# ywrt/slam-robot

Hardware: AMD Instinct MI355X
Metric: local-BA iters/sec (50 KF, 20k pts) (higher is better)
Workload: dtype f64

## Files before the change

slam-robot_amd/csrc/ba_chol.hip:

```cpp
#include "ba_lm.h"
#include "ba_tile.h"

namespace sg {

constexpr int kPanelWaves = 3;

__device__ __forceinline__ double& Wn(double* win, int i, int j) {
  return win[(i & (kCholWS - 1)) * kCholLd + (j & (kCholWS - 1))];
}

__device__ __forceinline__ double readlane_d(double v, int l) {
  const int lo = __builtin_amdgcn_readlane(__double2loint(v), l);
  const int hi = __builtin_amdgcn_readlane(__double2hiint(v), l);
  return __hiloint2double(hi, lo);
}



__device__ __forceinline__ void chol_diag16(double (&col)[kCholNb], int w, int lane, bool& bad) {
#pragma unroll
  for (int j = 0; j < kCholNb; ++j) {
    if (j < w) {
      const double piv = readlane_d(col[j], j);
      if (!(piv > 0.0)) bad = true;
// ... 848 lines not shown

struct TileSrc {
  int rev;
  int np;
  int sep;
  int nb;
  int ld;
};

__device__ __forceinline__ f64x4 tile_load(const double* __restrict__ S, int I, int J, int li, int lk,
                                           const TileSrc& ts) {
  f64x4 t;
  const int n = ts.nb, ld = ts.ld;
  const int cz = ld * ld + ld;
  const bool zsep = I >= ts.sep && J >= ts.sep;
#pragma unroll
  for (int q = 0; q < 4; ++q) {
    const int gi = 16 * I + lk + 4 * q, gj = 16 * J + li;
    const int si = ts.rev ? ts.np - 1 - gj : gi, sj = ts.rev ? ts.np - 1 - gi : gj;
    const bool in = I >= 0 && si < n && sj < n && !zsep;
    t[q] = S[in ? si * ld + sj : cz + ((gi == gj && !zsep) ? 1 : 0)];
  }
  return t;
}


__device__ __forceinline__ bool tile_diag(const f64x4& D, double ypart, TileShared& sh, double* zp, int K,
                                          int lane, int li, int lk) {
#pragma unroll
  for (int q = 0; q < 4; ++q) sh.Dw[(lk + 4 * q) * kTLd + li] = (lk + 4 * q <= li) ? D[q] : 0.0;
  const double ys = sum_rows4(ypart);
  if (lk == 0) sh.Yw[li] = ys;
  double ca[kCholNb];
#ifdef SG_X_NOFACTOR
  const bool bad = false;
#pragma unroll
  for (int r = 0; r < kCholNb; ++r) ca[r] = sh.Dw[r * kTLd + (lane & 15)];
#else
  const bool bad = tile_factor(sh.Dw, sh.Yw, sh.Id, sh.prw, ca);
#endif
  double* Zs = sh.Zs[K & 3];
  double* zk = sh.zK[K & 3];
  if (lane >= 16 && lane < 32) {
#pragma unroll
    for (int r = 0; r < kCholNb; ++r) Zs[r * kTLd + (lane - 16)] = ca[r];
  }
  if (lane == 32) {
#pragma unroll
    for (int r = 0; r < kCholNb; ++r) zk[r] = ca[r];
  }
  return bad;
}

__device__ __forceinline__ void tile_zp(const TileShared& sh, double* zp, int K, int lane, double* zg = nullptr) {
  if (lane < 16) {
    const double* Zs = sh.Zs[K & 3];
    const double* zk = sh.zK[K & 3];
    double s = 0.0;
#pragma unroll
    for (int r = 0; r < kCholNb; ++r) s = fma(Zs[r * kTLd + lane], zk[r], s);
    zp[16 * K + lane] = s;
  }
  if (zg) {
    const double* Zs = sh.Zs[K & 3];
    double* dst = zg + (size_t)K * kTB * 256;
#pragma unroll
    for (int e = lane; e < 256; e += 64) dst[e] = Zs[(e >> 4) * kTLd + (e & 15)];
  }
}

#define SG_TSTAMP(slot)                                                                  \
  if (kStamp && lane == 0) {                                                             \
    const unsigned long long now_ = __builtin_amdgcn_s_memtime();                       \
    tacc[slot] += now_ - tlast;                                                          \
    tlast = now_;                                                                        \
  }
#ifdef SG_X_ARRIVE
#define SG_PTRACE(K, slot) {}
#undef SG_TSTAMP
#define SG_TSTAMP(slot) {}
#define SG_AST(slot)                                                             \
  if (kStamp && lane == 0) {                                                     \
    const unsigned long long now_ = __builtin_amdgcn_s_memtime();               \
    tacc[slot] += now_ - tlast;                                                  \
    tlast = now_;                                                                \
  }
#else
#define SG_AST(slot) {}
#define SG_PTRACE(K, slot)                                                                  \
  if (kStamp && lane == 0 && (K) < kTraceK)                                                \
    d.stamps[64 + ((size_t)blockIdx.x * kTraceK + (K)) * 16 + (slot)] = __builtin_amdgcn_s_memtime();
#endif

__device__ __forceinline__ f64x4 tile_w(const f64x4& U, const double* Zs, int li, int lk) {
  const f64x4 zero = {0.0, 0.0, 0.0, 0.0};
  double zt[4];
#pragma unroll
  for (int s = 0; s < 4; ++s) zt[s] = Zs[(4 * s + lk) * kTLd + li];
  return mfma_f64_k16(zt, U, zero);
}
__device__ __forceinline__ void tile_w_store(const f64x4& Wt, double* __restrict__ Wg, int K, int J, int lane) {
  double* wg = Wg + ((size_t)K * kTB + (J - K)) * 256 + lane;
#pragma unroll
  for (int q = 0; q < 4; ++q) wg[q * 64] = Wt[q];
}

__device__ __forceinline__ void tile_rotate(f64x4 (&acc)[kTB]) {
  const f64x4 t = acc[0];
#pragma unroll
  for (int u = 0; u < kTB - 1; ++u) acc[u] = acc[u + 1];
  acc[kTB - 1] = t;
}

__device__ __forceinline__ void tile_col_load(f64x4 (&acc)[kTB], double& ypart, const Dev& d, int J, int K,
                                              int li, int lk, const TileSrc& ts) {
#pragma unroll
  for (int u = 0; u < kTB; ++u) acc[u] = tile_load(d.S, J - ((J - (u + K - 1)) & 7), J, li, lk, ts);
  const int gj = 16 * J + li, ld = ts.ld;
  const int sj = ts.rev ? ts.np - 1 - gj : gj;
  ypart = d.S[(lk == 0 && sj < ts.nb && J < ts.sep) ? ld * ld + sj : ld * ld + ld];
}

constexpr int kLaSpinMax = 1 << 20;
__device__ __forceinline__ bool la_done(const int* tend, int Kp) {
  return Kp >= 0 && Kp + 2 < tend[Kp];
}

template <bool kStamp>
__device__ __forceinline__ void tile_phase(f64x4 (&acc)[kTB], double& ypart, int& J, bool& late, bool& bad,
                                           bool& tmo, TileShared& sh, const Dev& d,
                                           double* __restrict__ Wg, double* zp, const int* tend, int K, int NT,
                                           int lane, int li, int lk, const TileSrc& ts, double* zg,
                                           unsigned long long (&tacc)[16], unsigned long long& tlast) {
  if (late) {
#ifdef SG_X_NOLATE
    J += kTB;
    late = false;
    return;
#endif
    const bool hasw = J < tend[K - 1];
    f64x4 Wt = {0.0, 0.0, 0.0, 0.0};
    if (hasw) Wt = tile_w(acc[0], sh.Zs[(K - 1) & 3], li, lk);
    SG_AST(0)
    const int Jw = J;
    J += kTB;
#ifndef SG_X_NOLOAD
    tile_col_load(acc, ypart, d, J, K, li, lk, ts);
#endif
    SG_AST(1)
    if (hasw) tile_w_store(Wt, Wg, K - 1, Jw, lane);
    SG_AST(2)
    tile_zp(sh, zp, K, lane, zg);
    SG_AST(3)
    late = false;
    SG_TSTAMP(13)
    return;
  }
  if (J == K + 1) SG_PTRACE(K, 8)
#ifdef SG_X_PRIO
  if (J == K + 1) __builtin_amdgcn_s_setprio(3);
#endif
#ifdef SG_X_IDLE
  if (J != K + 1) return;
#endif
#ifdef SG_X_NOTRAIL
  if (K >= 1 && J < tend[K - 1] && J == K + 1) {
#else
  if (K >= 1 && J < tend[K - 1]) {
#endif
    const double* Ub = sh.Ur[(K - 1) & 1][0];
    const bool own_la = J == K + 1 && la_done(tend, K - 1);
#pragma unroll
    for (int dd = 1; dd < kTB; ++dd) {
      if (K - 1 + dd <= J && !(dd == 2 && J == K + 1) && !(dd == 1 && own_la)) {
        double a[4];
#pragma unroll
        for (int s = 0; s < 4; ++s) a[s] = -Ub[(dd - 1) * 256 + s * 64 + lane];
        acc[dd] = mfma_f64_k16(a, acc[0], acc[dd]);
      }
    }
  }
  SG_TSTAMP(8)
  if (J == K + 1) { SG_AST(5) } else { SG_AST(10) }
  if (J == K + 1) SG_PTRACE(K, 9)
  const int te = tend[K];
  const bool act = J < te;
  const double* Zs = sh.Zs[K & 3];
  if (act) {
    const f64x4 zero = {0.0, 0.0, 0.0, 0.0};
    double za[4];
#pragma unroll
    for (int s = 0; s < 4; ++s) za[s] = Zs[li * kTLd + 4 * s + lk];
    const f64x4 U = mfma_f64_k16(za, acc[1], zero);
    acc[1] = U;
    double* ur = sh.Ur[K & 1][J - K - 1];
#pragma unroll
    for (int q = 0; q < 4; ++q) ur[q * 64 + lane] = U[q];
    if (J == K + 1) {
      __builtin_amdgcn_fence(__ATOMIC_RELEASE, "workgroup");
      if (lane == 0) __hip_atomic_store(&sh.uflag, K, __ATOMIC_RELAXED, __HIP_MEMORY_SCOPE_WORKGROUP);
    }
    const double* zk = sh.zK[K & 3];
#pragma unroll
    for (int q = 0; q < 4; ++q) ypart = fma(-U[q], zk[lk + 4 * q], ypart);
    if (J == K + 2) {
      double a[4];
#pragma unroll
      for (int s = 0; s < 4; ++s) a[s] = -U[s];
      acc[3] = mfma_f64_k16(a, U, acc[3]);
      if (la_done(tend, K)) {
        int spin = 0;
        while (__hip_atomic_load(&sh.uflag, __ATOMIC_RELAXED, __HIP_MEMORY_SCOPE_WORKGROUP) < K &&
               ++spin < kLaSpinMax)
          __builtin_amdgcn_s_sleep(0);
        tmo |= spin >= kLaSpinMax;
        __builtin_amdgcn_fence(__ATOMIC_ACQUIRE, "workgroup");
        const double* U1 = sh.Ur[K & 1][0];
        double b1[4];
#pragma unroll
        for (int s = 0; s < 4; ++s) b1[s] = -U1[s * 64 + lane];
        acc[2] = mfma_f64_k16(b1, U, acc[2]);
      }
    }
  }
  SG_TSTAMP(9)
  if (J == K + 1) { SG_AST(6) } else { SG_AST(11) }
  if (J == K + 1) {
    SG_PTRACE(K, 10)
    if (act) {
      double a[4];
#pragma unroll
      for (int s = 0; s < 4; ++s) a[s] = -acc[1][s];
      acc[2] = mfma_f64_k16(a, acc[1], acc[2]);
    }
    SG_TSTAMP(10)
    SG_AST(7)
    SG_PTRACE(K, 11)
    if (K + 1 < NT) {
      bad |= tile_diag(acc[2], ypart, sh, zp, K + 1, lane, li, lk);
    }
    SG_AST(8)
#ifdef SG_X_PRIO
    __builtin_amdgcn_s_setprio(0);
#endif
    SG_PTRACE(K, 12)
    late = true;
    SG_TSTAMP(11)
  } else if (act) {
    tile_w_store(tile_w(acc[1], Zs, li, lk), Wg, K, J, lane);
    SG_AST(12)
    SG_TSTAMP(12)
  }
}

__device__ __forceinline__ void tile_final(f64x4 (&acc)[kTB], int J, bool& late, TileShared& sh,
                                           double* __restrict__ Wg, const int* tend, int K, int lane, int li,
                                           int lk) {
  if (late) {
    if (J < tend[K - 1]) tile_w_store(tile_w(acc[0], sh.Zs[(K - 1) & 3], li, lk), Wg, K - 1, J, lane);
    late = false;
    return;
  }
  if (J < tend[K - 1]) {
    const double* Ub = sh.Ur[(K - 1) & 1][0];
    const bool own_la = J == K + 1 && la_done(tend, K - 1);
#pragma unroll
    for (int dd = 1; dd < kTB; ++dd) {
      if (K - 1 + dd <= J && !(dd == 2 && J == K + 1) && !(dd == 1 && own_la)) {
        double a[4];
#pragma unroll
        for (int s = 0; s < 4; ++s) a[s] = -Ub[(dd - 1) * 256 + s * 64 + lane];
        acc[dd] = mfma_f64_k16(a, acc[0], acc[dd]);
      }
    }
  }
}

__device__ __forceinline__ void sep_write(const f64x4 (&acc)[kTB], double ypart, int J, int ND, int NT, int m,
                                          int ns, double* __restrict__ sepb, double* __restrict__ sepy, int li,
                                          int lk) {
  if (J < ND || J >= ND + ns) return;
  const double ys = sum_rows4(ypart);
  const int Io = NT - 1 - J;
#pragma unroll
  for (int u = 0; u < kTB; ++u) {
    const int I = J - ((J - (u + ND - 1)) & 7);
    if (I >= ND) {
      double* dst = sepb + ((Io - m) * 7 + (NT - 1 - I - m)) * 256;
      const int C0 = 15 - li;
#pragma unroll
      for (int q = 0; q < 4; ++q) {
        const int Rd = C0, Cd = 15 - (lk + 4 * q);
        dst[(Rd >> 2) * 64 + Cd + 16 * (Rd & 3)] = acc[u][q];
      }
    }
  }
  if (lk == 0) sepy[(Io - m) * 16 + 15 - li] = ys;
}

__device__ __forceinline__ void sep_merge(f64x4 (&acc)[kTB], double& ypart, int J, int m, int ns,
                                          const double* __restrict__ sepb, const double* __restrict__ sepy,
                                          int lane, int li, int lk) {
  if (J < m || J >= m + ns) return;
#pragma unroll
  for (int u0 = 0; u0 < kTB; u0 += 2) {
    f64x4 t[2];
    bool use[2];
#pragma unroll
    for (int h = 0; h < 2; ++h) {
      const int u = u0 + h;
      const int I = J - ((J - (u + m - 2)) & 7);
      use[h] = I >= m;
      const double* src = sepb + (use[h] ? ((I - m) * 7 + (J - m)) * 256 : 0) + lane;
#pragma unroll
      for (int q = 0; q < 4; ++q) t[h][q] = src[q * 64];
    }
#pragma unroll
    for (int h = 0; h < 2; ++h)
      if (use[h])
#pragma unroll
        for (int q = 0; q < 4; ++q) acc[u0 + h][q] += t[h][q];
  }
  if (lk == 0) ypart += sepy[(J - m) * 16 + li];
}

template <int kCtrl>
__device__ __forceinline__ double dpp_mv(double v) {
  const int lo = __builtin_amdgcn_mov_dpp(__double2loint(v), kCtrl, 0xF, 0xF, false);
  const int hi = __builtin_amdgcn_mov_dpp(__double2hiint(v), kCtrl, 0xF, 0xF, false);
  return __hiloint2double(hi, lo);
}
__device__ __forceinline__ double bs_rowsum(const double (&p)[4], bool b0, bool b1) {
  const double k0 = b0 ? p[2] : p[0], k1 = b0 ? p[3] : p[1];
  const double s0 = b0 ? p[0] : p[2], s1 = b0 ? p[1] : p[3];
  const double a0 = k0 + dpp_mv<0xB1>(s0), a1 = k1 + dpp_mv<0xB1>(s1);
  const double k = b1 ? a1 : a0, sd = b1 ? a0 : a1;
  double v = k + dpp_mv<0x4E>(sd);
  v += dpp_mv<0x124>(v);
  v += dpp_mv<0x128>(v);
  return v;
}
__device__ __forceinline__ int bs_src_lane(int li) {
  const int q = li >> 2;
  return (((q >> 1) & 1) | ((q & 1) << 1)) + 16 * (li & 3);
}

__device__ __forceinline__ void tile_diag_pre(const f64x4& Z, double ypart, TileShared& sh, int li, int lk) {
  double* Zs = sh.Zs[0];
#pragma unroll
  for (int q = 0; q < 4; ++q) Zs[(lk + 4 * q) * kTLd + li] = Z[q];
  const double y = sum_rows4(ypart);
  double p[4];
#pragma unroll
  for (int q = 0; q < 4; ++q) p[q] = Z[q] * y;
  int lb = li;
  asm volatile("" : "+v"(lb));
  const double tot = bs_rowsum(p, (lb & 1) != 0, (lb & 2) != 0);
  if (li < 4) sh.zK[0][lk + 4 * (2 * (li & 1) + ((li >> 1) & 1))] = tot;
}

#ifndef SG_BS_BUF
#define SG_BS_BUF 2
#endif
constexpr int kBsBuf = SG_BS_BUF;
template <bool kRev>
__device__ __forceinline__ void bs_chain(const double* __restrict__ Wb, const double* zsrc, double* xs, int Khi,
                                         int Klo, double (&xw)[kTB - 1], int NT, int lane, int li, int lk) {
  auto wload = [&](double (&w)[kTB - 1][4], int K) {
#ifdef SG_X_BSHOT
    const double* src = Wb + (size_t)0 * (K >= 0 ? K : 0) + lane;
#else
    const double* src = Wb + (size_t)(K >= 0 ? K : 0) * kTB * 256 + lane;
#endif
#pragma unroll
    for (int dd = 1; dd < kTB; ++dd)
#pragma unroll
// ... 86 lines not shown
#pragma unroll
      for (int q = 0; q < 4; ++q) p[q] = fma(w[dd - 1][q], xw[dd - 1], p[q]);
#pragma unroll
    for (int q = 0; q < 4; ++q) {
      double v = p[q];
      v += dpp_d<0xB1>(v);
      v += dpp_d<0x4E>(v);
      v += dpp_d<0x141>(v);
      v += dpp_d<0x140>(v);
      p[q] = zk[q] - v;
    }
    unsigned long long mb = 0ull;
#pragma unroll
    for (int q = 0; q < 4; ++q) {
      int msk;
      asm volatile("v_bfe_i32 %0, %1, %2, 1" : "=v"(msk) : "v"(qbits), "n"(q));
      mb |= (unsigned long long)__double_as_longlong(p[q]) & (unsigned long long)(long long)msk;
    }
    const double xk = __shfl(__longlong_as_double((long long)mb), srcl);
    xat(K) = xk;
    asm volatile("" ::: "memory");
    if (lane == 0) __hip_atomic_store(done + K, 1, __ATOMIC_RELAXED, __HIP_MEMORY_SCOPE_WORKGROUP);
    xown = xk;
    wload(w, K - 4);
  };
  const int K0 = Khi - par;
  if (K0 < Klo) return;
  double wA[kTB - 1][4], wB[kTB - 1][4], zA[4], zB[4];
  wload(wA, K0);
  wload(wB, K0 - 2);
#pragma unroll
  for (int q = 0; q < 4; ++q) zA[q] = zsrc[16 * K0 + lk + 4 * q];
  int K = K0;
  bool first = true;
  for (; K >= Klo + 2; K -= 4) {
#pragma unroll
    for (int q = 0; q < 4; ++q) zB[q] = zsrc[16 * (K - 2) + lk + 4 * q];
    bs_row(K, wA, zA, first);
    first = false;
#pragma unroll
    for (int q = 0; q < 4; ++q) zA[q] = zsrc[16 * (K >= 4 ? K - 4 : 0) + lk + 4 * q];
    bs_row(K - 2, wB, zB, false);
  }
  if (K >= Klo) bs_row(K, wA, zA, first);
}

constexpr int kSepSpinMax = 1 << 22;
template <bool kStamp>
__global__ __launch_bounds__(kTileThreads) void k_chol_tiles(Dev d, const int32_t* panel_jend,
                                                             double* __restrict__ Wg, int32_t* tflag, int nd,
                                                             int flags) {
  const LmState* st = d.st;
  unsigned long long tlast = kStamp ? __builtin_amdgcn_s_memtime() : 0ull, tacc[16] = {};
  __shared__ TileShared sh;
  extern __shared__ double tdyn[];
  const bool border = (flags & 8) != 0;
  const int n = border ? d.kc0 : d.n, tid = threadIdx.x, lane = tid & 63;
  const int wave = __builtin_amdgcn_readfirstlane(tid >> 6);
  const int li = lane & 15, lk = lane >> 4;
  const int NT = (n + 15) >> 4;
  const bool bottom = nd > 0 && blockIdx.x == 1;
  const int nsf = (flags >> 8) & 15;
  const int ns = nsf > 0 && nsf < kTB ? nsf : kTB - 1;
  const int m = nd > 0 ? NT - nd - ns : NT;
  const int NTf = nd > 0 ? (bottom ? nd : m + ns) : NT;
  double* Wb = bottom ? Wg + (size_t)NT * kTB * 256 : Wg;
  double* zpg = Wg + (size_t)2 * NT * kTB * 256;
  double* sepb = zpg + 16 * NT;
  double* sepy = sepb + 49 * 256;
  const TileSrc ts{bottom ? 1 : 0, 16 * NT, bottom ? nd : (1 << 28), n, d.n};
  double* zg = border ? Wb : nullptr;
  double* xs = tdyn;
  double* zp = tdyn + 16 * NT;
  int* tend = reinterpret_cast<int*>(tdyn + 32 * NT);
  int* rdone = tend + NT;
  int* rdone_b = rdone + NT;
  for (int k = tid; k < 2 * NT; k += kTileThreads) rdone[k] = 0;
  const bool cand_lds = (flags & 2) != 0;
  CandLds cl;
  cl.carve(tdyn + 32 * NT + (3 * NT + 1) / 2, d.F, d.D, n);
  const int epoch = (nd > 0 && !bottom) ? tflag[1] : 0;
  if (tid == 0) {
    sh.fail = 0;
    sh.tmo = 0;
    sh.uflag = -1;
  }
  bool bad = false, tmo = false;
  const int spin_max = (flags & 4) ? 256 : kSepSpinMax;
  if (bottom && (flags & 4))
    for (int i = 0; i < 640; ++i) __builtin_amdgcn_s_sleep(127);
  const bool zpre_in = (flags & 16) != 0 && !bottom;
  f64x4 D0;
  bool zbad = false;
  if (zpre_in) {
#pragma unroll
    for (int q = 0; q < 4; ++q) D0[q] = d.zpre[(lk + 4 * q) * 16 + li];
    zbad = d.zpre[256] != 0.0;
  } else {
    D0 = tile_load(d.S, 0, 0, li, lk, ts);
  }
  double y0;
  {
    const int sj0 = ts.rev ? ts.np - 1 - li : li, ld = ts.ld;
    y0 = d.S[(lk == 0 && sj0 < n && 0 < ts.sep) ? ld * ld + sj0 : ld * ld + ld];
  }
  const int done = st->done;
  if (lane == 0) sh.simd[wave] = __builtin_amdgcn_s_getreg((1 << 11) | (4 << 6) | 4);
  for (int i = tid; i < 16 * kTLd; i += kTileThreads) sh.Id[i] = (i / kTLd == i % kTLd) ? 1.0 : 0.0;
  lds_barrier();
  int col = wave;
  {
    const int my = sh.simd[wave];
    int cnt[4] = {0, 0, 0, 0}, rank = 0;
#pragma unroll
    for (int w = 0; w < kTB; ++w) {
      const int sw = sh.simd[w] & 3;
      cnt[sw] += 1;
      if (w < wave && sw == my) rank += 1;
    }
#ifdef SG_X_PAIR4
    if (cnt[0] == 2 && cnt[1] == 2 && cnt[2] == 2 && cnt[3] == 2) col = my + 4 * rank;
#else
    if (cnt[0] == 2 && cnt[1] == 2 && cnt[2] == 2 && cnt[3] == 2) col = 2 * my + rank;
#endif
  }
  {
    f64x4 acc[kTB];
    double ypart = 0.0;
    int J = col;
    bool late = false;
    if (J == 0) J = kTB;
    tile_col_load(acc, ypart, d, J, 0, li, lk, ts);
    for (int k = tid; k < NT; k += kTileThreads) {
      if (!bottom) {
        tend[k] = min((panel_jend[k] + 15) >> 4, NTf);
      } else {
        const int c = NT - 1 - k;
        int te[kTB];
#pragma unroll
        for (int h = 0; h < kTB; ++h) te[h] = panel_jend[max(0, c - kTB + h)];
        int lo = c;
#pragma unroll
        for (int h = kTB - 1; h >= 0; --h) {
          const int i = c - kTB + h;
          if (i >= 0 && ((te[h] + 15) >> 4) > c) lo = i;
        }
        tend[k] = min(NT - lo, nd + ns);
      }
    }
    if (done) return;
    if (col == 0) {
      if (zpre_in) {
        tile_diag_pre(D0, y0, sh, li, lk);
        bad |= zbad;
      } else {
        bad |= tile_diag(D0, y0, sh, zp, 0, lane, li, lk);
      }
      tile_zp(sh, zp, 0, lane, zg);
    }
    else if (cand_lds)
      cand_prefetch(d, cl, st->cur, (col - 1) * 64 + lane, kTileThreads - 64);
    SG_TSTAMP(0)
    __syncthreads();
    SG_TSTAMP(1)
#ifdef SG_X_ARRIVE
    unsigned long long ar_sum[8] = {}, ar_max[8] = {}, ar_cnt[8] = {};
    unsigned long long t_ph = __builtin_amdgcn_s_memtime();
#endif
#pragma nounroll
    for (int K = 0; K < NTf; ++K) {
#ifdef SG_X_ARRIVE
      const int d0 = min(max(J - K, 0), 7);
      const int role = late ? 0 : (J == K + 1 ? 1 : 2);
#endif
      if (nd > 0 && !bottom && K == m - 1) {
        int spin = 0;
        while (__hip_atomic_load(tflag, __ATOMIC_RELAXED, __HIP_MEMORY_SCOPE_AGENT) <= epoch &&
               ++spin < spin_max)
          __builtin_amdgcn_s_sleep(1);
        __builtin_amdgcn_fence(__ATOMIC_ACQUIRE, "agent");
        tmo |= spin >= spin_max;
        sep_merge(acc, ypart, J, m, ns, sepb, sepy, lane, li, lk);
      }
      tile_phase<kStamp>(acc, ypart, J, late, bad, tmo, sh, d, Wb, zp, tend, K, NTf, lane, li, lk, ts, zg,
                         tacc, tlast);
      SG_TSTAMP(2)
      if (!late) tile_rotate(acc);
      SG_PTRACE(K, wave)
#ifdef SG_X_ARRIVE
      if (role == 0) { SG_AST(4) } else if (role == 1) { SG_AST(9) } else { SG_AST(13) }
      if (kStamp) {
        const unsigned long long ta = __builtin_amdgcn_s_memtime() - t_ph;
#pragma unroll
        for (int q = 0; q < 8; ++q)
          if (q == d0) {
            ar_sum[q] += ta;
            ar_max[q] = ar_max[q] > ta ? ar_max[q] : ta;
            ar_cnt[q] += 1;
          }
      }
#endif
      lds_barrier();
      if (late) tile_rotate(acc);
#ifdef SG_X_ARRIVE
      t_ph = __builtin_amdgcn_s_memtime();
      tlast = t_ph;
#endif
      SG_TSTAMP(3)
    }
#ifdef SG_X_ARRIVE
    if (kStamp && lane == 0) {
      unsigned long long* o = reinterpret_cast<unsigned long long*>(d.stamps) + kSegStamp + blockIdx.x * 256 + wave * 24;
#pragma unroll
      for (int q = 0; q < 8; ++q) {
        o[q] += ar_sum[q];
        o[8 + q] = o[8 + q] > ar_max[q] ? o[8 + q] : ar_max[q];
        o[16 + q] += ar_cnt[q];
      }
      unsigned long long* o2 = reinterpret_cast<unsigned long long*>(d.stamps) + kSegStamp + 512 + blockIdx.x * 256 +
                               wave * 16;
#pragma unroll
      for (int q = 0; q < 16; ++q) o2[q] += tacc[q];
    }
#endif
    if (bottom) {
      tile_final(acc, J, late, sh, Wb, tend, nd, lane, li, lk);
      sep_write(acc, ypart, J, nd, NT, m, ns, sepb, sepy, li, lk);
    }
  }
  if (bottom) {
    if (bad && lane == 0) sh.fail = 1;
    __syncthreads();
    for (int i = tid; i < 16 * nd; i += kTileThreads) zpg[i] = zp[i];
    if (tid == 0) zpg[16 * nd] = sh.fail ? 1.0 : 0.0;
    __builtin_amdgcn_fence(__ATOMIC_RELEASE, "agent");
    __syncthreads();
    if (tid == 0) {
      const int c = tflag[0];
      __hip_atomic_store(tflag, c + 1, __ATOMIC_RELEASE, __HIP_MEMORY_SCOPE_AGENT);
    }
    return;
  }
  if (nd > 0 && zpg[16 * nd] != 0.0) bad = true;
  if (bad && lane == 0) sh.fail = 1;
  __syncthreads();
  SG_TSTAMP(4)
  const int cur = st->cur;
  {
    double xw[kTB - 1];
#pragma unroll
    for (int dd = 0; dd < kTB - 1; ++dd) xw[dd] = 0.0;
    constexpr int kBs2Rows = 12;
    if (nd == 0) {
      if (NT >= kBs2Rows) {
        if (wave < 2) bs_chain2<false>(Wg, zp, xs, rdone, NT - 1, 0, xw, NT, wave, lane, li, lk, tmo);
      } else if (wave == 0) {
        bs_chain<false>(Wg, zp, xs, NT - 1, 0, xw, NT, lane, li, lk);
      }
    } else {
      if (wave == 0) bs_chain<false>(Wg, zp, xs, m + ns - 1, m, xw, NT, lane, li, lk);
      __syncthreads();
      if (wave < 2) {
#pragma unroll
        for (int dd = 1; dd < kTB; ++dd) xw[dd - 1] = dd <= ns ? xs[16 * (m - 1 + dd) + li] : 0.0;
        if (m >= kBs2Rows)
          bs_chain2<false>(Wg, zp, xs, rdone, m - 1, 0, xw, NT, wave, lane, li, lk, tmo);
        else if (wave == 0)
          bs_chain<false>(Wg, zp, xs, m - 1, 0, xw, NT, lane, li, lk);
      } else if (wave < 4) {
#pragma unroll
        for (int dd = 1; dd < kTB; ++dd) xw[dd - 1] = dd <= ns ? xs[16 * (NT - nd - dd) + 15 - li] : 0.0;
        if (nd >= kBs2Rows)
          bs_chain2<true>(Wg + (size_t)NT * kTB * 256, zpg, xs, rdone_b, nd - 1, 0, xw, NT, wave - 2, lane, li,
                          lk, tmo);
        else if (wave == 2)
          bs_chain<true>(Wg + (size_t)NT * kTB * 256, zpg, xs, nd - 1, 0, xw, NT, lane, li, lk);
      }
    }
  }
  if (tid == 0 && nd > 0) tflag[1] = epoch + 1;
  if (bad && lane == 0) sh.fail = 1;
  if (tmo && lane == 0) sh.tmo = 1;
  SG_TSTAMP(5)
  __syncthreads();
  double* y = d.work;
  for (int i = tid; i < n; i += kTileThreads) {
    d.xc[i] = xs[i];
    y[i] = xs[i];
  }
  if (border) {
    if (tid == 0) {
      d.xchg_chol[kCFail] = sh.fail ? 1.0 : 0.0;
      d.xchg_chol[kCTimeout] = sh.tmo ? 1.0 : 0.0;
    }
    return;
  }
  if (!cand_lds) __syncthreads();
  if (cand_lds)
    chol_candidates_lds<kTileThreads>(d, xs, sh.fail, cl, cur, sh.tmo);
  else
    chol_candidates<kTileThreads>(d, xs, sh.fail, sh.tmo);
  SG_TSTAMP(6)
  if (kStamp && lane == 0 && wave < 2)
    for (int s_ = 0; s_ < 16; ++s_) d.stamps[16 * wave + s_] += tacc[s_];
}
#undef SG_TSTAMP

template <bool kQlds>
__global__ __launch_bounds__(kBordThreads) void k_chol_border(Dev d, double* __restrict__ Wg, int flags) {
  const LmState* st = d.st;
  if (st->done) return;
  extern __shared__ double bdyn[];
  const int n = d.n, nf = d.kc0, nk = n - nf, NT = (nf + 15) >> 4;
  const int tid = threadIdx.x, lane = tid & 63, wave = tid >> 6, li = lane & 15, lk = lane >> 4;
  const bool cand_lds = (flags & 2) != 0;
  double* xs = bdyn;
  double* zq = bdyn + 16 * NT;
  int* rdone = reinterpret_cast<int*>(bdyn + 32 * NT);
  size_t off = 32 * (size_t)NT + (NT + 1) / 2;
  constexpr bool qlds = kQlds;
  double* Ql = bdyn + off;
  double* Qg = Wg + (size_t)NT * kTB * 256;
  if (qlds) off += 256 * (size_t)NT;
  CandLds cl;
  cl.carve(bdyn + off, d.F, d.D, n);
  const double* S = d.S;
  const double* xc = d.xc;
  __shared__ double Cs[16][kTLd];
  __shared__ double rk[16], xk[16], rpart[kBordThreads / 64][16];
  __shared__ double Ids[16 * kTLd], prw[2 * kCholNb];
  for (int i = tid; i < 16 * kTLd; i += kBordThreads) Ids[i] = (i / kTLd == i % kTLd) ? 1.0 : 0.0;
  __shared__ int bad_sh;
  unsigned long long tst[10];
  auto now_t = []() {
    unsigned long long t;
    asm volatile("s_memtime %0\n\ts_waitcnt lgkmcnt(0)" : "=s"(t) : : "memory");
    return t;
  };
  tst[0] = now_t();
  auto bstamp = [&](int k) { tst[k + 1] = now_t(); };
  for (int k = 1; k < 10; ++k) tst[k] = tst[0];
  const int fail0 = d.xchg_chol[kCFail] != 0.0, tmo0 = d.xchg_chol[kCTimeout] != 0.0;
  for (int k = tid; k < NT; k += kBordThreads) rdone[k] = 0;
  if (tid == 0) bad_sh = fail0;
  __shared__ double vring[8][256], wring[4][256], fring[2][4][256];
  __shared__ int vpost, fpost[2], wdone;
  if (tid == 0) {
    vpost = -1;
    fpost[0] = fpost[1] = -1;
    wdone = -1;
  }
  __syncthreads();
  bool tmo_chain = false;
  auto wait_ge = [&](int* flag, int v) {
    int spin = 0;
    while (__hip_atomic_load(flag, __ATOMIC_RELAXED, __HIP_MEMORY_SCOPE_WORKGROUP) < v && ++spin < kLaSpinMax)
      __builtin_amdgcn_s_sleep(0);
// ... 298 lines not shown
```

slam-robot_amd/csrc/ba_plan.cpp:

```cpp
#include "ba_plan.h"

#include <algorithm>
#include <climits>
#include <utility>

#include "common.h"

namespace sg {


void PlanBlocks(const sg_problem& p, Order* o) {
  o->F = p.num_frames;
  o->P = p.num_points;
  o->M = p.num_obs;
  o->D = p.num_dist;
  o->frame_block.assign(o->F, -1);
  o->NB = 0;
  for (int f = 0; f < o->F; ++f)
    if (p.frame_rot_free[f] || p.frame_trans_free[f]) o->frame_block[f] = o->NB++;
  o->nk = p.cameras_free ? 7 * p.num_cameras : 0;
  o->n = 6 * o->NB + o->nk;
}

void PlanPointOrder(const sg_problem& p, Order* o) {
// ... 484 lines not shown
  std::vector<int32_t> panel_bend(std::max(npanel, 1), 0);
  for (int pk = 0; pk < npanel; ++pk) {
    const int row_hi = std::min(n, (pk + 1) * kCholNb) - 1;
    const int blk_hi = row_hi / 6;
    int jmax = (pk + 1) * kCholNb;
    for (int b = 0; b < NB; ++b)
      if (lo_blk[b] <= blk_hi) jmax = std::max(jmax, 6 * b + 6);
    jmax = std::min(jmax, n);
    panel_jmax[pk] = std::min(n, (jmax + kCholNb - 1) / kCholNb * kCholNb);
    if (nk) {
      panel_bend[pk] = std::min(jmax, 6 * NB);
      panel_jmax[pk] = n;
    }
  }
  if (nk) panel_jmax.insert(panel_jmax.end(), panel_bend.begin(), panel_bend.end());
  e.pack_off.assign(npanel + 1, 0);
  for (int pk = 0; pk < npanel; ++pk)
    e.pack_off[pk + 1] = e.pack_off[pk] + std::min(kCholNb, n - pk * kCholNb) * (panel_jmax[pk] - pk * kCholNb);
  e.npack = (size_t)e.pack_off[npanel] + n;
  e.band_tiles = 0;
  for (int pk = 0; pk < npanel; ++pk)
    e.band_tiles = std::max(e.band_tiles, (panel_jmax[pk] + kCholNb - 1) / kCholNb - pk);
  std::vector<int32_t>&stile = e.stile, &s_loff = e.s_loff, &s_lidx = e.s_lidx;
  const int nft = (6 * NB + kCholNb - 1) / kCholNb;
  std::vector<int32_t> row_off(nft + 1, 0), cend(nft, 0);
  for (int R = 0; R < nft; ++R) {
    cend[R] = std::min(nft, (panel_jmax[R] + kCholNb - 1) / kCholNb);
    row_off[R + 1] = row_off[R] + std::max(0, cend[R] - R);
    for (int C = R; C < cend[R]; ++C) stile.push_back((R << 16) | C);
  }
  std::vector<std::vector<int32_t>> tl(stile.size());
  for (int s = 0; s < nseg; ++s) {
    const SchurSeg& sg = segs[s];
    for (int u = 0; u < sg.ntw * (sg.ntw + 1) / 2; ++u) {
      const int R = sg.t0 + schur_tile_r(u), C = sg.t0 + schur_tile_c(u);
      if (R < nft && C < cend[R]) tl[row_off[R] + C - R].push_back(sg.s_off + 256 * u);
    }
  }
  size_t smax = 0;
  for (const auto& l : tl) smax = std::max(smax, l.size());
  e.s_lstride = (int)std::max<size_t>(256, (smax + 255) / 256 * 256);
  s_lidx.assign(std::max<size_t>(tl.size(), 1) * e.s_lstride, 0);
  for (size_t t = 0; t < tl.size(); ++t) {
    s_loff.push_back((int)tl[t].size());
    std::copy(tl[t].begin(), tl[t].end(), s_lidx.begin() + t * e.s_lstride);
  }
  e.nstile = (int)stile.size();
  if (stile.empty()) stile.push_back(0);
  if (s_loff.empty()) s_loff.push_back(0);
  return e;
}


CholPlan PlanChol(const Order& o, const Envelope& e, const CholGrants& g, const LoadKnobs& k) {
  const int F = o.F, D = o.D, n = o.n, NB = o.NB, nk = o.nk, npanel = e.npanel;
  const std::vector<int32_t>& panel_jmax = e.panel_jmax;
  CholPlan c;
  c.gstage = (size_t)std::max(n, 1) * 8 * (1 + kCholNb) <= g.global && k.chol_gstage;
  c.window = npanel <= kJendSh;
  for (int pk = 0; pk < npanel; ++pk)
    if (panel_jmax[pk] - pk * kCholNb > kCholWS) c.window = false;
  c.tiles = n > 0 && nk == 0 && npanel <= kTileMaxNT && !k.chol_window;
  for (int pk = 0; pk < npanel; ++pk)
    if ((panel_jmax[pk] + kCholNb - 1) / kCholNb - pk > kTB) c.tiles = false;
  c.border = false;
  if (nk > 0 && NB > 0 && n - 6 * NB <= kCholNb && !k.chol_window && k.chol_border) {
    const int32_t* panel_bend = panel_jmax.data() + npanel;
    const int ntf = (6 * NB + kCholNb - 1) / kCholNb;
    c.border = ntf <= kTileMaxNT;
    for (int pk = 0; pk < ntf; ++pk)
      if ((panel_bend[pk] + kCholNb - 1) / kCholNb - pk > kTB) c.border = false;
    if (c.border) {
      c.tiles = true;
      c.border_flags = 0;
      for (int f : {1, 2, 3})
        if (border_lds_doubles(ntf, f, F, D, n) * sizeof(double) <= g.border &&
            (!(f & 2) || (F <= kCandMax && D <= kCandMax)))
          c.border_flags = f;
    }
  }
  c.nd = 0;
  c.ns = kTB - 1;
  if (c.tiles && !c.border && npanel >= kSplitMinNT && k.chol_split) {
    const bool fixed7 = k.chol_sep7;
    double best = 1e30;
    int reach = 0;
    for (int m = 1; m < npanel; ++m) {
      reach = std::max(reach, std::min(npanel, (panel_jmax[m - 1] + kCholNb - 1) / kCholNb));
      const int ns = fixed7 ? kTB - 1 : reach - m;
      const int nd = npanel - m - ns;
      if (ns < 1 || ns > kTB - 1 || reach - m > ns || nd < 2) continue;
      const double cost = std::max((double)m, nd + 2.5) + ns;
      if (cost < best) {
        best = cost;
        c.nd = nd;
        c.ns = ns;
      }
    }
  }
  if (c.tiles) {
    c.wg_size = (size_t)2 * npanel * kTB * 256 + 16 * (size_t)npanel + 49 * 256 + 7 * 16 + 2;
    c.tile_lds = (size_t)npanel * 32 * sizeof(double) + (size_t)(3 * npanel + 1) / 2 * sizeof(double);
    c.cand_lds = !c.border && F <= kCandMax && D <= kCandMax &&
                 c.tile_lds + cand_lds_bytes(F, D, n) <= 100 * 1024 &&
                 c.tile_lds + cand_lds_bytes(F, D, n) <= g.tiles;
    if (c.cand_lds) c.tile_lds += cand_lds_bytes(F, D, n);
    if (c.tile_lds > g.tiles) {
      c.tiles = false;
      c.border = false;
      c.nd = 0;
    }
  }
  return c;
}

}
```

slam-robot_amd/csrc/ba_solver.h:

```cpp
#ifndef SG_BA_SOLVER_H_
#define SG_BA_SOLVER_H_

#include <hip/hip_runtime.h>

#include <cstdlib>
#include <chrono>
#include <memory>
#include <string>
#include <vector>

#include "ba_kernels.h"
#include "ba_plan.h"
#include "common.h"
#include "dbuf.h"
#include "hostio.h"
#include "hostmirror.h"

namespace sg {

void ValidateProblem(const sg_problem* p);

class Comm;

class BaSolver {
// ... 5 lines not shown
  void Reserve(int F, int P, int M);
  void Begin(const sg_solver_options& o);
  void Iterate(int n);
  void Sweep(int n);
  void Sync();
  void Summary(sg_solver_summary* s);
  void Download(sg_problem* p);
  void Solve(const sg_solver_options& o, sg_problem* p, sg_solver_summary* s);
  void Evaluate(double* residuals, double* cost, int32_t* nfail);
  void SetTiming(bool on);
  int KernelTimes(char* names, int names_len, double* ms, int32_t* counts, int max);
  int KernelWork(double* bytes, double* flops, int max);
  void CommInit(const void* id128, int nranks, int rank);
  void CommInitLocal(std::shared_ptr<struct LocalGroup> g, int rank);
  void CommInitHost(int nranks, int rank, int (*fn)(double*, long long, int, void*), void* user);
  static void UniqueId(void* id128);

  void Info(sg_ba_info* out) const;

  double ReprojectMap(sg_map* m);

  hipStream_t stream() const { return stream_; }
  int nranks() const;

 private:
  sg_device_options dev_;
  hipStream_t stream_ = nullptr;
  HostMirror mb_;
  void ReadState(LmState* h);
  void WaitStream(hipStream_t s);
  hipEvent_t ev_wait_ = nullptr;
  void EnqueueIterations(int n);
  hipEvent_t dev_marks_[5] = {nullptr, nullptr, nullptr, nullptr, nullptr};
  hipEvent_t ev_idle_ = nullptr;
  hipEvent_t ev_idle_prev_ = nullptr;
  std::chrono::steady_clock::time_point idle_host_;
  bool idle_valid_ = false;
  void MarkIdle(hipStream_t s);
  void DevMark(hipStream_t s, int i);
  std::string LoadDeviceTimes(std::chrono::steady_clock::time_point load_t0, bool idle_valid_prev,
                              double idle_gap_host);
  bool need_seq_ = true;
  std::unique_ptr<Comm> comm_;
  bool loaded_ = false;
  bool began_ = false;
  CholPlan chol_;
  WorkCounts wk_;
  EnvCounts env_;
  size_t border_lds_max_ = 0;
  DBuf<double> Wg_;
  DBuf<int32_t> tflag_;
  bool chol_force_tmo_ = getenv("SG_CHOL_FORCE_TIMEOUT") && atoi(getenv("SG_CHOL_FORCE_TIMEOUT")) != 0;
  bool chol_zpre_off_ = getenv("SG_CHOL_ZPRE") && atoi(getenv("SG_CHOL_ZPRE")) == 0;
  bool pack_force_ = getenv("SG_PACK_S") != nullptr;
  bool spec_ = !(getenv("SG_SPEC") && atoi(getenv("SG_SPEC")) == 0);
  size_t jslot_ = 0, cslot_ = 0;
  int merge_ = getenv("SG_XCHG_MERGE") ? (std::string(getenv("SG_XCHG_MERGE")) == "force" ? 2 : atoi(getenv("SG_XCHG_MERGE")) != 0)
                                       : 1;
  size_t ntail_ = 0;
  bool pending_decision_ = false;
  int32_t nallreduce_ = 0;
  bool comm_force_ = getenv("SG_COMM_FORCE") && atoi(getenv("SG_COMM_FORCE")) == 1;
  bool stamp_on_ = false;
  int ncu_ = 256;
  size_t tile_lds_set_ = 0;
  size_t gchol_lds_max_ = 0;
  std::unique_ptr<class Stager> stager_;
  DBuf<unsigned long long> stamps_;

 public:
  std::vector<unsigned long long> Stamps();

 private:
  int F_ = 0, P_ = 0, M_ = 0, NB_ = 0, n_ = 0, D_ = 0, ncam_ = 0;
  std::vector<int32_t> point_perm_;
  std::vector<int32_t> obs_perm_;
  struct StructKey {
    int32_t ncam = -1, cams_free = 0, F = -1, P = -1, M = -1, D = -1;
    std::vector<int32_t> frame_camera, obs_frame, obs_point, dist_frame, dist_prev;
    std::vector<uint8_t> rot_free, trans_free, point_free;
  } skey_;
  int32_t full_loads_ = 0, value_loads_ = 0;
  bool SameStructure(const sg_problem& p) const;
  void SaveStructure(const sg_problem& p);
  void LoadValues(const sg_problem& p);
  void ResetState(hipStream_t s);

 public:
  void LoadCounts(int32_t* full, int32_t* values) const {
    *full = full_loads_;
    *values = value_loads_;
  }

 private:
  DBuf<LmState> st_;
  DBuf<double> k_, q_, t_, X_, obs_pt_, J_, V_, g_, scale_p_, diag_p_, Vinv_, tp_, scale_c_, diag_c_, camdiag_,
      camg_, cam_slab_, S_slab_, chunk_scal_, cam_wide_, S_wide_, xchg_cam_, S_, rhs_, xchg_upd_,
      xchg_chol_, work_, fd_r_, fd_J_, fd_D_, fd_X_, red_, zpre_;
  DBuf<int32_t> frame_cam_, frame_block_, poff_, obs_frame_, fd_a_, fd_b_, fd_boff_, fd_bidx_, cam_loff_,
      cam_lidx_, s_loff_, s_lidx_, r_loff_, r_lidx_, mobs_frame_, mobs_point_, mframe_cam_;
  DBuf<uint8_t> rot_free_, trans_free_, pfree_, obs_fixed_;
  DBuf<int32_t> work_i_;
  DBuf<int32_t> fd_pair_;
  DBuf<int32_t> pu_units_;
  DBuf<int32_t> pack_off_;
  DBuf<double> Spk_;
// ... 43 lines not shown
```

slam-robot_amd/csrc/ba_solver.hip:

```cpp
#include <hip/hip_runtime.h>

#include <chrono>
#include <string>
#include <thread>

#include <algorithm>
#include <cfloat>
#include <cmath>
#include <cstring>
#include <cstdlib>
#include <numeric>

#include "ba_solver.h"
#include "ba_device.h"
#include "ba_launch.h"
#include "comm.h"
#include "stager.h"

namespace sg {

__global__ __launch_bounds__(256) void k_copy_u64(const unsigned long long* __restrict__ src,
                                                  unsigned long long* __restrict__ dst, size_t n) {
  for (size_t i = (size_t)blockIdx.x * blockDim.x + threadIdx.x; i < n; i += (size_t)gridDim.x * blockDim.x)
    dst[i] = src[i];
// ... 811 lines not shown
          TimedLaunchEnd(kKDecide);
        }
        pending_decision_ = false;
      }
    } else {
      TimedLaunchBegin(kKCamReduce);
      LaunchCamReduceK(NB_ + 1, stream_, d, 0);
      TimedLaunchEnd(kKCamReduce);
    }
    if (!merged) AllReduceSum(xchg_cam_.ptr, (size_t)nv + kXNum + nranks());
    if (nk_) {
      LaunchIntrLinearizeK(stream_, d, n_, nk_, NB_, ncam_, M_, wk_.intr_nsl);
    }
    if (!fin_in_schur && !fin1_in_schur) {
      TimedLaunchBegin(kKCamFinal);
      LaunchCamFinalizeK(stream_, d, merged ? 1 : 0, decide_in_fin ? 1 : 0);
      TimedLaunchEnd(kKCamFinal);
    }
    TimedLaunchBegin(kKSchur);
    LaunchSchurK(std::max(wk_.nseg, 1), wk_.nwide, fin_in_schur ? 1 : (fin1_in_schur ? 2 : 0), stream_, d);
    TimedLaunchEnd(kKSchur);
    TimedLaunchBegin(kKSReduce);
    const int nwv = env_.nstile + NB_;
    const int samode = merged ? 2 : (d.assemble ? 1 : 0);
    const bool zpre = chol_.tiles && !chol_.border && nk_ == 0 && samode == 1 && !(multi_x || merged) && !chol_zpre_off_;
    LaunchSReduceK(std::max(nwv, 1), stream_, d, samode, zpre ? 1 : 0);
    TimedLaunchEnd(kKSReduce);
    if (nk_) {
      LaunchIntrSchurK(stream_, d, n_, nk_, NB_, ncam_, P_, wk_.intr_nsl);
    }
    if (multi_x || pack_force_ || merged) {
      const int npanel = (n_ + kCholNb - 1) / kCholNb;
      const dim3 pg(npanel + 1, 4);
      TimedLaunchBegin(kKXchg);
      LaunchSPackK(pg, stream_, S_.ptr, n_, (const int32_t*)work_i_.ptr, (const int32_t*)pack_off_.ptr, npanel,
                   Spk_.ptr, 0);
      AllReduceSum(Spk_.ptr, env_.npack + (merged ? ntail_ : 0));
      if (fin1_in_schur)
        LaunchSUnpackFinK(pg, stream_, d, (const int32_t*)work_i_.ptr, (const int32_t*)pack_off_.ptr, npanel,
                          Spk_.ptr);
      else
        LaunchSPackK(pg, stream_, S_.ptr, n_, (const int32_t*)work_i_.ptr, (const int32_t*)pack_off_.ptr, npanel,
                     Spk_.ptr, 1);
      TimedLaunchEnd(kKXchg);
      if (merged && !fin1_in_schur) {
        TimedLaunchBegin(kKCamFinal);
        LaunchCamFinalizeK(stream_, d, 2, 0);
        TimedLaunchEnd(kKCamFinal);
      }
    }
    TimedLaunchBegin(kKChol);
    if (chol_.tiles)
      LaunchCholTiles(d.stamps != nullptr, dim3(chol_.nd > 0 ? 2 : 1), d,
                      (chol_.cand_lds ? 2 : 0) | (chol_force_tmo_ ? 4 : 0) | (zpre ? 16 : 0));
    else if (chol_.window)
      LaunchCholWindowK(d.stamps != nullptr, stream_, d, (const int32_t*)work_i_.ptr, rdg_.ptr);
    else
      LaunchCholGlobalK(chol_.gstage, (size_t)std::max(n_, 1) * 8 * (chol_.gstage ? 1 + kCholNb : 1), stream_, d,
                        (const int32_t*)work_i_.ptr, rdg_.ptr);
    TimedLaunchEnd(kKChol);
    if (nk_) LaunchIntrStepK(stream_, d);
    TimedLaunchBegin(kKPointUpd);
    if (spec_) {
      LaunchUpdateLin(d);
    } else {
      LaunchPointUpdateK(std::max(wk_.npu, 1), stream_, d);
    }
    TimedLaunchEnd(kKPointUpd);
    const bool multi = comm_ && comm_->nranks() > 1;
    const bool decide_in_reduce = !multi && nk_ == 0 && merge_ != 2;
    TimedLaunchBegin(kKUpdRed);
    if (spec_)
      LaunchCamReduceK(NB_ + 2, stream_, d, decide_in_reduce ? 2 : 1);
    else
      LaunchUpdReduceK(stream_, d, multi ? 0 : 1);
    TimedLaunchEnd(kKUpdRed);
    if (multi) AllReduceSum(xchg_upd_.ptr, kUNum);
    if (spec_) {
      pending_decision_ = !decide_in_reduce;
    } else if (multi) {
      TimedLaunchBegin(kKDecide);
      LaunchDecideK(stream_, d, 0);
      TimedLaunchEnd(kKDecide);
    }
  }
  if (pending_decision_) {
    TimedLaunchBegin(kKDecide);
    LaunchDecideK(stream_, d, 1);
    TimedLaunchEnd(kKDecide);
    pending_decision_ = false;
  }
  SG_HIP_CHECK(hipGetLastError());
}

__global__ void k_force_linearize(LmState* st) {
  if (threadIdx.x == 0) {
    st->need_lin = 1;
    st->done = 0;
  }
}

void BaSolver::Sweep(int n) {
  SG_REQUIRE(loaded_, SG_EINVAL, "no problem loaded");
  SG_HIP_CHECK(hipSetDevice(dev_.device));
  Dev d = MakeDev();
  for (int it = 0; it < n; ++it) {
    hipLaunchKernelGGL(k_force_linearize, dim3(1), dim3(64), 0, stream_, st_.ptr);
// ... 227 lines not shown
```

Measured before the change: 8062.

## Streamline bottom-to-top Cholesky handoff with write-through stores and epoch flag

The bottom block of the split tile Cholesky now writes its z vector, W tiles, separator tiles and failure flags straight to global memory with agent-scope relaxed atomic stores as it computes them. This replaces the trailing copy loop, the release fence and the read-modify-write of the flag. The top block spins on the flag with lane 0 only, and only for the separator columns that need it, then reads with relaxed atomic loads. Waves 2 and 3 issue an acquire fence before the back-substitution. The planner's handoff cost constant drops from 2.5 to 2.25 and ties now prefer a smaller separator. Timing-only stamp hooks and optional delay flags are added, and the memory ordering now rests on vmcnt waits and relaxed atomics instead of release/acquire pairs, which could be fragile.

```diff
diff --git a/slam-robot_amd/csrc/ba_chol.hip b/slam-robot_amd/csrc/ba_chol.hip
--- a/slam-robot_amd/csrc/ba_chol.hip
+++ b/slam-robot_amd/csrc/ba_chol.hip
@@ -924,7 +924,15 @@
   return bad;
 }
 
-__device__ __forceinline__ void tile_zp(const TileShared& sh, double* zp, int K, int lane, double* zg = nullptr) {
+__device__ __forceinline__ void st_wt(double* p, double v) {
+  __hip_atomic_store(p, v, __ATOMIC_RELAXED, __HIP_MEMORY_SCOPE_AGENT);
+}
+__device__ __forceinline__ double ld_wt(const double* p) {
+  return __hip_atomic_load(p, __ATOMIC_RELAXED, __HIP_MEMORY_SCOPE_AGENT);
+}
+
+__device__ __forceinline__ void tile_zp(const TileShared& sh, double* zp, int K, int lane, double* zg = nullptr,
+                                        double* zw = nullptr) {
   if (lane < 16) {
     const double* Zs = sh.Zs[K & 3];
     const double* zk = sh.zK[K & 3];
@@ -932,6 +940,7 @@
 #pragma unroll
     for (int r = 0; r < kCholNb; ++r) s = fma(Zs[r * kTLd + lane], zk[r], s);
     zp[16 * K + lane] = s;
+    if (zw) st_wt(zw + 16 * K + lane, s);
   }
   if (zg) {
     const double* Zs = sh.Zs[K & 3];
@@ -960,9 +969,16 @@
 #else
 #define SG_AST(slot) {}
 #define SG_PTRACE(K, slot)                                                                  \
-  if (kStamp && lane == 0 && (K) < kTraceK)                                                \
+  if (kStamp && lane == 0 && (K) < kTraceK - 1)                                            \
     d.stamps[64 + ((size_t)blockIdx.x * kTraceK + (K)) * 16 + (slot)] = __builtin_amdgcn_s_memtime();
 #endif
+#define SG_HSTAMP(i)                                                 \
+  if (kStamp && lane == 0) {                                         \
+    const unsigned long long now_ = __builtin_amdgcn_s_memtime();   \
+    hacc[i] = now_ - hlast;                                          \
+    hlast = now_;                                                    \
+  }
+constexpr int kHoStamp = 64 + (kTraceK - 1) * 16;
 
 __device__ __forceinline__ f64x4 tile_w(const f64x4& U, const double* Zs, int li, int lk) {
   const f64x4 zero = {0.0, 0.0, 0.0, 0.0};
@@ -971,10 +987,16 @@
   for (int s = 0; s < 4; ++s) zt[s] = Zs[(4 * s + lk) * kTLd + li];
   return mfma_f64_k16(zt, U, zero);
 }
-__device__ __forceinline__ void tile_w_store(const f64x4& Wt, double* __restrict__ Wg, int K, int J, int lane) {
+__device__ __forceinline__ void tile_w_store(const f64x4& Wt, double* __restrict__ Wg, int K, int J, int lane,
+                                             bool wt) {
   double* wg = Wg + ((size_t)K * kTB + (J - K)) * 256 + lane;
-#pragma unroll
-  for (int q = 0; q < 4; ++q) wg[q * 64] = Wt[q];
+  if (wt) {
+#pragma unroll
+    for (int q = 0; q < 4; ++q) st_wt(wg + q * 64, Wt[q]);
+  } else {
+#pragma unroll
+    for (int q = 0; q < 4; ++q) wg[q * 64] = Wt[q];
+  }
 }
 
 __device__ __forceinline__ void tile_rotate(f64x4 (&acc)[kTB]) {
@@ -1002,8 +1024,9 @@
 __device__ __forceinline__ void tile_phase(f64x4 (&acc)[kTB], double& ypart, int& J, bool& late, bool& bad,
                                            bool& tmo, TileShared& sh, const Dev& d,
                                            double* __restrict__ Wg, double* zp, const int* tend, int K, int NT,
-                                           int lane, int li, int lk, const TileSrc& ts, double* zg,
+                                           int lane, int li, int lk, const TileSrc& ts, double* zg, double* zw,
                                            unsigned long long (&tacc)[16], unsigned long long& tlast) {
+  const bool wt = zw != nullptr;
   if (late) {
 #ifdef SG_X_NOLATE
     J += kTB;
@@ -1020,9 +1043,9 @@
     tile_col_load(acc, ypart, d, J, K, li, lk, ts);
 #endif
     SG_AST(1)
-    if (hasw) tile_w_store(Wt, Wg, K - 1, Jw, lane);
+    if (hasw) tile_w_store(Wt, Wg, K - 1, Jw, lane, wt);
     SG_AST(2)
-    tile_zp(sh, zp, K, lane, zg);
+    tile_zp(sh, zp, K, lane, zg, zw);
     SG_AST(3)
     late = false;
     SG_TSTAMP(13)
@@ -1119,7 +1142,7 @@
     late = true;
     SG_TSTAMP(11)
   } else if (act) {
-    tile_w_store(tile_w(acc[1], Zs, li, lk), Wg, K, J, lane);
+    tile_w_store(tile_w(acc[1], Zs, li, lk), Wg, K, J, lane, wt);
     SG_AST(12)
     SG_TSTAMP(12)
   }
@@ -1129,7 +1152,7 @@
                                            double* __restrict__ Wg, const int* tend, int K, int lane, int li,
                                            int lk) {
   if (late) {
-    if (J < tend[K - 1]) tile_w_store(tile_w(acc[0], sh.Zs[(K - 1) & 3], li, lk), Wg, K - 1, J, lane);
+    if (J < tend[K - 1]) tile_w_store(tile_w(acc[0], sh.Zs[(K - 1) & 3], li, lk), Wg, K - 1, J, lane, true);
     late = false;
     return;
   }
@@ -1163,11 +1186,11 @@
 #pragma unroll
       for (int q = 0; q < 4; ++q) {
         const int Rd = C0, Cd = 15 - (lk + 4 * q);
-        dst[(Rd >> 2) * 64 + Cd + 16 * (Rd & 3)] = acc[u][q];
-      }
-    }
-  }
-  if (lk == 0) sepy[(Io - m) * 16 + 15 - li] = ys;
+        st_wt(dst + (Rd >> 2) * 64 + Cd + 16 * (Rd & 3), acc[u][q]);
+      }
+    }
+  }
+  if (lk == 0) st_wt(sepy + (Io - m) * 16 + 15 - li, ys);
 }
 
 __device__ __forceinline__ void sep_merge(f64x4 (&acc)[kTB], double& ypart, int J, int m, int ns,
@@ -1185,7 +1208,7 @@
       use[h] = I >= m;
       const double* src = sepb + (use[h] ? ((I - m) * 7 + (J - m)) * 256 : 0) + lane;
 #pragma unroll
-      for (int q = 0; q < 4; ++q) t[h][q] = src[q * 64];
+      for (int q = 0; q < 4; ++q) t[h][q] = ld_wt(src + q * 64);
     }
 #pragma unroll
     for (int h = 0; h < 2; ++h)
@@ -1193,7 +1216,7 @@
 #pragma unroll
         for (int q = 0; q < 4; ++q) acc[u0 + h][q] += t[h][q];
   }
-  if (lk == 0) ypart += sepy[(J - m) * 16 + li];
+  if (lk == 0) ypart += ld_wt(sepy + (J - m) * 16 + li);
 }
 
 template <int kCtrl>
@@ -1386,6 +1409,9 @@
                                                              int flags) {
   const LmState* st = d.st;
   unsigned long long tlast = kStamp ? __builtin_amdgcn_s_memtime() : 0ull, tacc[16] = {};
+  const unsigned long long hstart = tlast;
+  unsigned long long hlast = 0ull, hacc[6] = {};
+  bool hchain = false;
   __shared__ TileShared sh;
   extern __shared__ double tdyn[];
   const bool border = (flags & 8) != 0;
@@ -1413,7 +1439,7 @@
   const bool cand_lds = (flags & 2) != 0;
   CandLds cl;
   cl.carve(tdyn + 32 * NT + (3 * NT + 1) / 2, d.F, d.D, n);
-  const int epoch = (nd > 0 && !bottom) ? tflag[1] : 0;
+  const int epoch = nd > 0 ? tflag[bottom ? 0 : 1] : 0;
   if (tid == 0) {
     sh.fail = 0;
     sh.tmo = 0;
@@ -1423,6 +1449,8 @@
   const int spin_max = (flags & 4) ? 256 : kSepSpinMax;
   if (bottom && (flags & 4))
     for (int i = 0; i < 640; ++i) __builtin_amdgcn_s_sleep(127);
+  if (bottom && (flags & 64))
+    for (int i = 0; i < 16; ++i) __builtin_amdgcn_s_sleep(127);
   const bool zpre_in = (flags & 16) != 0 && !bottom;
   f64x4 D0;
   bool zbad = false;
@@ -1490,7 +1518,7 @@
       } else {
         bad |= tile_diag(D0, y0, sh, zp, 0, lane, li, lk);
       }
-      tile_zp(sh, zp, 0, lane, zg);
+      tile_zp(sh, zp, 0, lane, zg, bottom ? zpg : nullptr);
     }
     else if (cand_lds)
       cand_prefetch(d, cl, st->cur, (col - 1) * 64 + lane, kTileThreads - 64);
@@ -1508,16 +1536,27 @@
       const int role = late ? 0 : (J == K + 1 ? 1 : 2);
 #endif
       if (nd > 0 && !bottom && K == m - 1) {
-        int spin = 0;
-        while (__hip_atomic_load(tflag, __ATOMIC_RELAXED, __HIP_MEMORY_SCOPE_AGENT) <= epoch &&
-               ++spin < spin_max)
-          __builtin_amdgcn_s_sleep(1);
-        __builtin_amdgcn_fence(__ATOMIC_ACQUIRE, "agent");
-        tmo |= spin >= spin_max;
-        sep_merge(acc, ypart, J, m, ns, sepb, sepy, lane, li, lk);
+        if (flags & 128)
+          for (int i = 0; i < 16; ++i) __builtin_amdgcn_s_sleep(127);
+        if (kStamp) hlast = __builtin_amdgcn_s_memtime();
+        if (J >= m && J < m + ns) {
+          int spin = 0;
+          if (lane == 0)
+            while (__hip_atomic_load(tflag, __ATOMIC_RELAXED, __HIP_MEMORY_SCOPE_AGENT) <= epoch &&
+                   ++spin < spin_max)
+              __builtin_amdgcn_s_sleep(1);
+          spin = __builtin_amdgcn_readfirstlane(spin);
+          asm volatile("" ::: "memory");
+          SG_HSTAMP(0)
+          tmo |= spin >= spin_max;
+          sep_merge(acc, ypart, J, m, ns, sepb, sepy, lane, li, lk);
+          if (kStamp) asm volatile("s_waitcnt vmcnt(0)" ::: "memory");
+          SG_HSTAMP(1)
+          hchain = J == m;
+        }
       }
       tile_phase<kStamp>(acc, ypart, J, late, bad, tmo, sh, d, Wb, zp, tend, K, NTf, lane, li, lk, ts, zg,
-                         tacc, tlast);
+                         bottom ? zpg : nullptr, tacc, tlast);
       SG_TSTAMP(2)
       if (!late) tile_rotate(acc);
       SG_PTRACE(K, wave)
@@ -1558,24 +1597,33 @@
     }
 #endif
     if (bottom) {
+      if (kStamp) {
+        hlast = __builtin_amdgcn_s_memtime();
+        hacc[5] = hlast - hstart;
+      }
+      if (lane == 0) st_wt(zpg + 16 * nd + wave, bad ? 1.0 : 0.0);
       tile_final(acc, J, late, sh, Wb, tend, nd, lane, li, lk);
       sep_write(acc, ypart, J, nd, NT, m, ns, sepb, sepy, li, lk);
+      SG_HSTAMP(0)
     }
   }
   if (bottom) {
-    if (bad && lane == 0) sh.fail = 1;
+    SG_HSTAMP(1)
+    asm volatile("s_waitcnt vmcnt(0)" ::: "memory");
     __syncthreads();
-    for (int i = tid; i < 16 * nd; i += kTileThreads) zpg[i] = zp[i];
-    if (tid == 0) zpg[16 * nd] = sh.fail ? 1.0 : 0.0;
-    __builtin_amdgcn_fence(__ATOMIC_RELEASE, "agent");
-    __syncthreads();
-    if (tid == 0) {
-      const int c = tflag[0];
-      __hip_atomic_store(tflag, c + 1, __ATOMIC_RELEASE, __HIP_MEMORY_SCOPE_AGENT);
+    SG_HSTAMP(2)
+    if (tid == 0) __hip_atomic_store(tflag, epoch + 1, __ATOMIC_RELAXED, __HIP_MEMORY_SCOPE_AGENT);
+    SG_HSTAMP(3)
+    if (kStamp && tid == 0) {
+      unsigned long long* o = d.stamps + kHoStamp + kTraceK * 16;
+#pragma unroll
+      for (int i = 0; i < 4; ++i) o[i] += hacc[i];
+      o[4] += 1;
+      o[5] += hacc[5];
     }
     return;
   }
-  if (nd > 0 && zpg[16 * nd] != 0.0) bad = true;
+  if (nd > 0 && __any(lane < kTB && ld_wt(zpg + 16 * nd + (lane & (kTB - 1))) != 0.0)) bad = true;
   if (bad && lane == 0) sh.fail = 1;
   __syncthreads();
   SG_TSTAMP(4)
@@ -1592,7 +1640,10 @@
         bs_chain<false>(Wg, zp, xs, NT - 1, 0, xw, NT, lane, li, lk);
       }
     } else {
-      if (wave == 0) bs_chain<false>(Wg, zp, xs, m + ns - 1, m, xw, NT, lane, li, lk);
+      if (wave == 0)
+        bs_chain<false>(Wg, zp, xs, m + ns - 1, m, xw, NT, lane, li, lk);
+      else if (wave == 2 || wave == 3)
+        __builtin_amdgcn_fence(__ATOMIC_ACQUIRE, "agent");
       __syncthreads();
       if (wave < 2) {
 #pragma unroll
@@ -1637,6 +1688,11 @@
   SG_TSTAMP(6)
   if (kStamp && lane == 0 && wave < 2)
     for (int s_ = 0; s_ < 16; ++s_) d.stamps[16 * wave + s_] += tacc[s_];
+  if (kStamp && lane == 0 && hchain) {
+    d.stamps[kHoStamp + 0] += hacc[0];
+    d.stamps[kHoStamp + 1] += hacc[1];
+    d.stamps[kHoStamp + 2] += 1;
+  }
 }
 #undef SG_TSTAMP
 
diff --git a/slam-robot_amd/csrc/ba_plan.cpp b/slam-robot_amd/csrc/ba_plan.cpp
--- a/slam-robot_amd/csrc/ba_plan.cpp
+++ b/slam-robot_amd/csrc/ba_plan.cpp
@@ -560,6 +560,8 @@
 }
 
 
+constexpr double kHandoffPhases = 2.25;
+
 CholPlan PlanChol(const Order& o, const Envelope& e, const CholGrants& g, const LoadKnobs& k) {
   const int F = o.F, D = o.D, n = o.n, NB = o.NB, nk = o.nk, npanel = e.npanel;
   const std::vector<int32_t>& panel_jmax = e.panel_jmax;
@@ -598,8 +600,8 @@
       const int ns = fixed7 ? kTB - 1 : reach - m;
       const int nd = npanel - m - ns;
       if (ns < 1 || ns > kTB - 1 || reach - m > ns || nd < 2) continue;
-      const double cost = std::max((double)m, nd + 2.5) + ns;
-      if (cost < best) {
+      const double cost = std::max((double)m, nd + kHandoffPhases) + ns;
+      if (cost < best || (cost == best && ns < c.ns)) {
         best = cost;
         c.nd = nd;
         c.ns = ns;
diff --git a/slam-robot_amd/csrc/ba_solver.h b/slam-robot_amd/csrc/ba_solver.h
--- a/slam-robot_amd/csrc/ba_solver.h
+++ b/slam-robot_amd/csrc/ba_solver.h
@@ -81,6 +81,10 @@
   DBuf<int32_t> tflag_;
   bool chol_force_tmo_ = getenv("SG_CHOL_FORCE_TIMEOUT") && atoi(getenv("SG_CHOL_FORCE_TIMEOUT")) != 0;
   bool chol_zpre_off_ = getenv("SG_CHOL_ZPRE") && atoi(getenv("SG_CHOL_ZPRE")) == 0;
+  int chol_delay_ = !getenv("SG_CHOL_DELAY") ? 0
+                    : std::string(getenv("SG_CHOL_DELAY")) == "bottom" ? 64
+                    : std::string(getenv("SG_CHOL_DELAY")) == "top"    ? 128
+                                                                       : 0;
   bool pack_force_ = getenv("SG_PACK_S") != nullptr;
   bool spec_ = !(getenv("SG_SPEC") && atoi(getenv("SG_SPEC")) == 0);
   size_t jslot_ = 0, cslot_ = 0;
diff --git a/slam-robot_amd/csrc/ba_solver.hip b/slam-robot_amd/csrc/ba_solver.hip
--- a/slam-robot_amd/csrc/ba_solver.hip
+++ b/slam-robot_amd/csrc/ba_solver.hip
@@ -887,7 +887,7 @@
     TimedLaunchBegin(kKChol);
     if (chol_.tiles)
       LaunchCholTiles(d.stamps != nullptr, dim3(chol_.nd > 0 ? 2 : 1), d,
-                      (chol_.cand_lds ? 2 : 0) | (chol_force_tmo_ ? 4 : 0) | (zpre ? 16 : 0));
+                      (chol_.cand_lds ? 2 : 0) | (chol_force_tmo_ ? 4 : 0) | (zpre ? 16 : 0) | chol_delay_);
     else if (chol_.window)
       LaunchCholWindowK(d.stamps != nullptr, stream_, d, (const int32_t*)work_i_.ptr, rdg_.ptr);
     else
```

New measurement: 8174, median of 6. 1.4% higher.
